# NWC-CUAHSI-Summer-Institute/LGAR-py

Hardware: AMD Instinct MI355X
Metric: column-timesteps/sec (higher is better)
Workload: dtype f32

## Files before the change

lgar_py_amd/csrc/lgar_column.hpp:

```cpp
#pragma once
#include "lgar_geff.hpp"

namespace lgar {

template <typename R> struct Glob {
  R dt_h, initial_psi, pdm, wp_psi, frozen;
  R giuh[LGAR_GMAX];
  int nint, nsub, ng, bottom_mode, closed_form;
  long long iter_cap;
};

#define LGAR_COOP_GROUPS 16
template <typename S, int FMAX, int STRIDE = WAVE> struct FrontsView {
  S *base;
  unsigned char *fl;
  __device__ __forceinline__ S &Z(int i) const { return base[(0 * FMAX + i) * STRIDE]; }
  __device__ __forceinline__ S &TH(int i) const { return base[(1 * FMAX + i) * STRIDE]; }
  __device__ __forceinline__ S &PS(int i) const { return base[(2 * FMAX + i) * STRIDE]; }
  __device__ __forceinline__ S &DZ(int i) const { return base[(3 * FMAX + i) * STRIDE]; }
  __device__ __forceinline__ unsigned char &flag(int i) const { return fl[i * STRIDE]; }
  __device__ __forceinline__ int layer(int i) const { return fl[i * STRIDE] & 0x7f; }
  __device__ __forceinline__ bool bottom(int i) const { return (fl[i * STRIDE] & LGAR_FLAG_BOTTOM) != 0; }
  __device__ __forceinline__ void set_flag(int i, int layer, bool bottom) const {
    fl[i * STRIDE] = (unsigned char)(layer | (bottom ? LGAR_FLAG_BOTTOM : 0));
  }
  __device__ __forceinline__ void copy(int dst, int src) const {
    Z(dst) = Z(src); TH(dst) = TH(src); PS(dst) = PS(src); DZ(dst) = DZ(src);
    fl[dst * STRIDE] = fl[src * STRIDE];
  }
};

constexpr int MODE_LITERAL = 0, MODE_FAST = 1, MODE_MIXED = 3, MODE_COOP = 4, MODE_MIXED_COOP = 6;

template <typename S, int MODE> struct ModeTraits : ScalarKind<S> {
  using K = ScalarKind<S>;
  static constexpr bool literal = MODE == MODE_LITERAL;
  static constexpr bool mixed = MODE == MODE_MIXED || MODE == MODE_MIXED_COOP;
  static constexpr bool coop = MODE == MODE_COOP || MODE == MODE_MIXED_COOP;
  static constexpr bool mixed_f64 = mixed && K::plain_f64;
  static constexpr bool coop_f64 = coop && K::plain_f64;
  static constexpr int pol = (literal && K::f64) ? POL_LIBRARY : (!literal && K::plain_f32) ? POL_RCP32 : mixed_f64 ? POL_MIXED : POL_LEAN;
  static constexpr int stride = coop ? LGAR_COOP_GROUPS : WAVE;
  static constexpr bool giuh_mem = MODE == MODE_MIXED && !K::dual;
  static constexpr bool late_forcing_sums = MODE == MODE_MIXED;
  static constexpr bool fused_walk = !literal && !coop;
};

template <typename S, int NL, int FMAX, int MODE> struct Column {
  using R = real_t<S>;
  using M = ModeTraits<S, MODE>;
  static constexpr int POL = M::pol;
  const ColParams<S, NL> &P;
  const LGAR_KARG Glob<R> *G;
  FrontsView<S, FMAX, M::stride> F;
  int nf;
  int status;
  S ponded_water, previous_precip, ending_volume;
  S giuh_q[LGAR_GMAX];
  static constexpr int DEAD = LGAR_ST_BOTTOM | LGAR_ST_OVERFLOW | LGAR_ST_STRUCT;
  R *giuh_mem = nullptr;
  size_t giuh_stride = 0;
  bool giuh_live = false;
  S k_deepest;
  bool new_front_frozen;
  S memo_theta, memo_g;
  int memo_layer = -1;
  unsigned near_sat_fronts = 0u;
  S post_mass;
  bool post_mass_valid = false;
  bool post_event = false;
  bool psi_rewritten = false;
  S aet_psi_wp_memo;
  bool aet_psi_wp_known = false;
  bool count_geff = false;
  int share_lanes = 0;
  R *xchg = nullptr;
  int coop_rank = 0;
  int cap = FMAX;
  S a_precip, a_pet, a_aet, a_infil, a_runoff, a_perc, a_giuh, a_disch;

  __device__ Column(const ColParams<S, NL> &p, const LGAR_KARG Glob<R> *g, const FrontsView<S, FMAX, M::stride> &f) : P(p), G(g), F(f) {}

  __device__ __forceinline__ S cum_at(int k) const { return sel<S, NL>(P.cum, k); }
  __device__ __forceinline__ S capillary_drive(const LayerK<S> &lk, S theta1, S theta2, int site = 0, CoopRiders *riders = nullptr) {
    (void)site; (void)riders;
    LGAR_MEASURE_POINT(NOGEFF, lk, theta1, theta2)
    LGAR_COUNT_GEFF_CALL(site)
    LGAR_MEASURE_POINT(DUP_GEFF, lk, theta1, theta2)
    if constexpr (M::literal && M::f64) {
      return G->closed_form ? geff_closed<S, POL>(lk, theta1, theta2) : geff_literal<S, POL>(lk, theta1, theta2, G->nint);
    }
    if constexpr (M::dual && M::f64 && !M::literal) {
      if (share_lanes >= 2 && !G->closed_form) return geff_fused<S>(lk, theta1, theta2, G->nint, xchg, share_lanes);
    }
    if constexpr (M::coop_f64 && !M::mixed) {
      if (share_lanes > 1 && !G->closed_form) return geff_fused<S>(lk, theta1, theta2, G->nint, xchg, share_lanes, coop_rank, riders);
    }
    if constexpr (M::coop_f64 && M::mixed) {
      if (share_lanes > 1 && !G->closed_form)
        return geff_mixed_coop(val(lk.alpha), val(lk.n), val(lk.m), val(lk.inv_m), val(lk.inv_n), val(lk.ksat), val(lk.te), val(lk.tr),
                               theta1, theta2, G->nint, xchg, share_lanes, coop_rank);
    }
    if constexpr (M::mixed_f64) {
      if (!G->closed_form)
        return geff_mixed(val(lk.alpha), val(lk.n), val(lk.m), val(lk.inv_m), val(lk.inv_n), val(lk.ksat), val(lk.te), val(lk.tr),
                          theta1, theta2, G->nint);
    }
    return G->closed_form ? geff_closed<S, POL>(lk, theta1, theta2) : geff(lk, theta1, theta2, G->nint);
  }
  __device__ __forceinline__ double capillary_drive_fronts(const LayerK<double> &lk, double theta1, double theta2, double psi1,
                                                           double psi2, double &kr_end) {
    LGAR_MEASURE_POINT(NOGEFF_FRONTS, lk, theta1, theta2, kr_end)
    LGAR_COUNT_GEFF_CALL(1)
    if constexpr (M::coop && M::mixed) {
      if (share_lanes > 1) return geff_mixed_heads<true>(lk, theta1, theta2, psi1, psi2, G->nint, kr_end, xchg, share_lanes, coop_rank);
    }
    return geff_mixed_heads(lk, theta1, theta2, psi1, psi2, G->nint, kr_end);
  }
  __device__ __forceinline__ S cum_prev(int k) const {
    S r = S(R(0.0));
#pragma unroll
    for (int j = 0; j < NL - 1; j++) {
      const S cj = P.cum[j];
      r = choose(k == j + 1, cj, r);
    }
    return r;
  }

  __device__ __forceinline__ bool feq(int a, int b) const {
    return val(F.Z(a)) == val(F.Z(b)) && val(F.PS(a)) == val(F.PS(b)) && val(F.DZ(a)) == val(F.DZ(b));
  }
  __device__ __forceinline__ void fdel(int i) {
    for (int j = i; j < nf - 1; j++) F.copy(j, j + 1);
    nf--;
  }
  __device__ __forceinline__ void range_of(int k, int &lo, int &len) const {
    lo = -1; len = 0;
    for (int i = 0; i < nf; i++)
      if (F.layer(i) == k) { if (len == 0) lo = i; len++; }
  }

  static constexpr int SCAN = 8;
  struct Rows {
    R z[SCAN], th[SCAN];
    int fl[SCAN];
  };
  __device__ __forceinline__ void fetch_rows(Rows &r) const {
#pragma unroll
    for (int q = 0; q < SCAN; q++) {
      r.z[q] = val(F.Z(q));
      r.th[q] = val(F.TH(q));
      r.fl[q] = F.flag(q);
    }
  }

  __device__ __forceinline__ S mass_balance() const {
    S ls[NL];
    if constexpr (M::coop_f64) {
      if (nf <= SCAN) {
        Rows r;
        fetch_rows(r);
#pragma unroll
        for (int j = 0; j < NL; j++) ls[j] = S(R(0.0));
#pragma unroll
        for (int q = 0; q < SCAN; q++) {
          const bool on = q < nf;
          const int lay = r.fl[q] & 0x7f;
          const bool next_same = (q + 1 < nf) && ((r.fl[(q + 1 < SCAN) ? q + 1 : q] & 0x7f) == lay);
          const R dth = next_same ? r.th[q] - r.th[(q + 1 < SCAN) ? q + 1 : q] : r.th[q];
          R base = R(0.0);
#pragma unroll
          for (int j = 1; j < NL; j++) base = choose(lay == j, val(P.cum[j]) - val(P.thick[j]), base);
          const R term = (r.z[q] - base) * dth;
#pragma unroll
          for (int j = 0; j < NL; j++) ls[j] = choose(on && lay == j, ls[j] + term, ls[j]);
        }
        S tot = ls[NL - 1];
#pragma unroll
        for (int j = NL - 2; j >= 0; j--) tot = ls[j] + tot;
        return tot;
      }
    }
    int i = 0;
#pragma unroll
    for (int j = 0; j < NL; j++) {
      S base = (j == 0) ? S(R(0.0)) : P.cum[j] - P.thick[j];
      S sum = S(R(0.0));
      while (i < nf && F.layer(i) == j) {
        bool next_same = (i + 1 < nf) && (F.layer(i + 1) == j);
        S dth = next_same ? (F.TH(i) - F.TH(i + 1)) : F.TH(i);
        sum = sum + (F.Z(i) - base) * dth;
// ... 1051 lines not shown
            riders.n = 1 + k;
            riders.l = le;
            riders.se = se_from_theta(le, th_e);
#pragma unroll
            for (int q = 0; q < LGAR_LMAX; q++) riders.k[q] = R(1.0);
            g = capillary_drive(lk, theta_1, theta_2, 1, &riders);
            ki = riders.k[0];
            if (i == 0 && new_front_frozen) ki = ki * G->frozen;
            fronts_done = true;
          }
        }
        LGAR_MEASURE_POINT(F32_HEADS_FROM_PSI, lk, i, g, ki, fronts_done)
        if (!fronts_done) {
          g = capillary_drive(lk, theta_1, theta_2, 1);
          ki = front_k(i, lk);
        }
        if (is_nan(val(g))) status |= LGAR_ST_NAN;
        S dzdt;
        if (k == 0) {
          dzdt = dv<POL>(S(R(1.0)), delta_theta) * (dv<POL>(lk.ksat * (g + h_p), F.Z(i)) + ki);
        } else {
          S den = S(R(0.0)) + dv<POL>(F.Z(i) - cum_prev(k), ki);
#pragma unroll
          for (int j = 0; j < NL - 1; j++)
            if (j < k) {
              const LayerK<S> lj = pick_static(P, j);
              S kl;
              bool rode = false;
              if constexpr (M::coop_f64 && !M::mixed) {
                if (riders.n > 0) { kl = riders.k[1 + j]; rode = true; }
              }
              if (!rode) {
                S tl = theta_from_h<S, POL>(lj, F.PS(i));
                kl = k_from_se<S, POL>(lj, se_from_theta(lj, tl));
              }
              S pt = (j != 0) ? P.cum[(j > 0) ? j - 1 : 0] : S(R(0.0));
              den = den + dv<POL>(P.cum[j] - pt, kl);
            }
          dzdt = dv<POL>(S(R(1.0)), delta_theta) * (dv<POL>(F.Z(i), den) + dv<POL>(lk.ksat * (g + h_p), F.Z(i)));
        }
        F.DZ(i) = dzdt;
        LGAR_MEASURE_POINT(CLK, 17)
      }
    }
  }

  __device__ __forceinline__ S calc_dry_depth() {
    const LayerK<S> l0 = pick_static(P, 0);
    S delta_theta = l0.te - F.TH(0);
    S tau = G->dt_h * l0.ksat / delta_theta;
    S g = capillary_drive(l0, F.TH(0), l0.te, 2);
    if (is_nan(val(g))) status |= LGAR_ST_NAN;
    S dry = R(0.5) * (tau + sq(tau * tau + R(4.0) * tau * g));
    return mn(P.cum[0], dry);
  }

  __device__ __forceinline__ void create_surficial_front(S dry_depth, S &ponded, S &infiltration) {
    if (nf >= cap) { status |= LGAR_ST_OVERFLOW; return; }
    const LayerK<S> l0 = pick_static(P, 0);
    S cur_theta = F.TH(0);
    S delta_theta = l0.te - cur_theta;
    S theta_new;
    bool to_bottom = false;
    if (val(dry_depth * delta_theta) > val(ponded)) {
      infiltration = ponded;
      theta_new = mn((cur_theta + ponded / dry_depth), l0.te);
      ponded = S(R(0.0));
    } else {
      infiltration = dry_depth * delta_theta;
      ponded = ponded - (dry_depth * delta_theta);
      theta_new = l0.te;
      to_bottom = !(val(dry_depth) < val(P.cum[0]));
    }
    for (int j = nf; j > 0; j--) F.copy(j, j - 1);
    nf++;
    F.Z(0) = dry_depth;
    F.TH(0) = theta_new;
    F.set_flag(0, 0, to_bottom);
    F.PS(0) = h_from_se<S, POL>(l0, se_from_theta(l0, theta_new));
    new_front_frozen = true;
    F.DZ(0) = S(R(0.0));
  }

  __device__ __forceinline__ void insert_water(int fdd, S precip, S &ponded, S &infiltration, S &runoff) {
    const R dt = G->dt_h;
    S h_p = (ponded - precip) * dt;
    if (val(h_p) < R(0.0)) h_p = S(R(0.0));
    const int kfp = F.layer(fdd);
    int lo, len;
    range_of(kfp, lo, len);
    const int nxt_i = lo + 1;
    if (nxt_i >= nf && (nf != NL || G->bottom_mode == 0)) { status |= LGAR_ST_STRUCT; return; }
    const LayerK<S> lk = pick(P, kfp);
    S g = S(R(0.0));
    if (nf != NL) {
      const S theta_1 = F.TH(nxt_i < nf ? nxt_i : nf - 1);
      bool hit = memo_layer == kfp && same_bits(theta_1, memo_theta);
      if constexpr (M::dual) {
        if (share_lanes >= 2) {
          const bool value_hit = memo_layer == kfp && val(theta_1) == val(memo_theta);
          if (any_lane(value_hit && !hit) != 0ull) hit = false;
        }
      }
      if (hit) {
        g = memo_g;
      } else {
        g = capillary_drive(lk, theta_1, lk.te, 3);
        memo_theta = theta_1; memo_g = g; memo_layer = kfp;
      }
    }
    if (is_nan(val(g))) status |= LGAR_ST_NAN | LGAR_ST_NEGBASE;
    S f_p;
    if (kfp == 0) {
      f_p = P.ksat[0] * (R(1.0) + dv<POL>(g + h_p, F.Z(fdd)));
    } else {
      S fd_ksat = lk.ksat * G->frozen;
      S bottom_sum = dv<POL>(F.Z(fdd) - cum_prev(kfp), fd_ksat);
      bottom_sum = bottom_sum + dv<POL>(P.cum[0] - R(0.0), P.ksat[0] * G->frozen);
#pragma unroll
      for (int j = 1; j < NL - 1; j++)
        if (j < kfp) {
          const LayerK<S> lj = pick_static(P, j);
          S tl = theta_from_h<S, POL>(lj, F.PS(fdd));
          S kl = k_from_se<S, POL>(lj, se_from_theta(lj, tl));
          bottom_sum = bottom_sum + dv<POL>(P.cum[j] - P.cum[j - 1], kl);
        }
      f_p = dv<POL>(F.Z(fdd), bottom_sum) + dv<POL>((g + h_p) * fd_ksat, F.Z(fdd));
    }
    S pond_temp = ponded - f_p * dt;
    if (val(pond_temp) < R(0.0)) pond_temp = S(R(0.0));
    S fp_cm = f_p * dt;
    if (G->pdm > R(0.0)) {
      if (val(pond_temp) < G->pdm) {
        infiltration = mn(ponded, fp_cm);
        ponded = ponded - infiltration;
      } else if (val(pond_temp) > G->pdm) {
        ponded = S(G->pdm);
        infiltration = fp_cm;
      }
      S r = pond_temp - G->pdm;
      runoff = (val(r) > R(0.0)) ? r : S(R(0.0));
    } else {
      infiltration = mn(ponded, fp_cm);
      S r = ponded - infiltration;
      ponded = S(G->pdm);
      runoff = (val(r) > R(0.0)) ? r : S(R(0.0));
    }
  }

  __device__ __forceinline__ void init_state() {
    nf = NL;
    status = 0;
    new_front_frozen = false;
#pragma unroll
    for (int k = 0; k < NL; k++) {
      const LayerK<S> lk = pick_static(P, k);
      F.Z(k) = P.cum[k];
      F.TH(k) = theta_from_h<S, POL>(lk, S(G->initial_psi));
      F.PS(k) = S(G->initial_psi);
      if (k == NL - 1) k_deepest = k_from_se<S, POL>(lk, se_from_theta(lk, F.TH(k)));
      F.DZ(k) = S(R(0.0));
      F.set_flag(k, k, true);
    }
    ponded_water = previous_precip = S(R(0.0));
#pragma unroll
    for (int i = 0; i < LGAR_GMAX; i++) giuh_q[i] = S(R(0.0));
    ending_volume = mass_balance();
    drain();
  }

  __device__ __forceinline__ void drain() {
    a_precip = a_pet = a_aet = a_infil = a_runoff = a_perc = a_giuh = a_disch = S(R(0.0));
  }

  __device__ __forceinline__ void forward(S precip, S pet) {
    const R dt = G->dt_h;
    if (is_nan(val(precip)) || is_nan(val(pet))) status |= LGAR_ST_NAN;
    S ending_volume_sub = ending_volume;
    for (int sub = 0; sub < G->nsub; sub++) {
      if (status & DEAD) return;
      new_front_frozen = false;
      post_mass_valid = false;
      S precip_sub = precip * dt;
      S pet_sub = pet * dt;
      S ponded_depth_sub = precip_sub + ponded_water;
      S ponded_water_sub = S(R(0.0)), runoff_sub = S(R(0.0)), infiltration_sub = S(R(0.0)), AET_sub = S(R(0.0));
      const bool create = (val(previous_precip) == R(0.0)) && (val(precip_sub) > R(0.0)) && (val(ponded_water) == R(0.0));
      LGAR_MEASURE_POINT(CLK, 0)
      LGAR_MEASURE_POINT(DUP_FDD)
      const int fdd = free_drainage_front();
      const bool saturated = val(F.TH(0)) >= val(P.te[0]);
      if (val(pet) > R(0.0)) {
        if (!aet_psi_wp_known) {
          aet_psi_wp_memo = aet_psi_wp<S, POL>(pick_static(P, 0), G->wp_psi);
          aet_psi_wp_known = true;
        }
        AET_sub = aet_from_psi_wp<S, POL>(pet, dt, F.PS(0), aet_psi_wp_memo);
      }
      if constexpr (!M::late_forcing_sums) {
        a_precip = a_precip + precip_sub;
        a_pet = a_pet + ((val(pet_sub) > R(0.0)) ? pet_sub : S(R(0.0)));
      }
      const bool inserting = !create && val(ponded_depth_sub) > R(0.0);
      LGAR_MEASURE_POINT(CLK, 1)
      if (inserting) {
        LGAR_ABLATABLE(INSERT, insert_water(fdd, precip_sub, ponded_depth_sub, infiltration_sub, runoff_sub);)
        a_infil = a_infil + infiltration_sub;
        a_runoff = a_runoff + runoff_sub;
        ponded_water_sub = ponded_depth_sub;
      }
      LGAR_MEASURE_POINT(CLK, 2)
      if (!create || !saturated) {
        S perc_sub = S(R(0.0));
        LGAR_ABLATABLE(MOVE, perc_sub = move_wetting_front(create ? S(R(0.0)) : infiltration_sub, AET_sub, ending_volume_sub, fdd);)
        if (!create) a_perc = a_perc + perc_sub;
      }
      if (__builtin_expect(create && !saturated, 0)) {
        S dry_depth = calc_dry_depth();
        create_surficial_front(dry_depth, ponded_depth_sub, infiltration_sub);
        a_infil = a_infil + infiltration_sub;
        post_mass_valid = false;
      }
      if (!inserting) {
        if (val(ponded_depth_sub) < G->pdm) {
          runoff_sub = S(R(0.0));
          ponded_water_sub = ponded_depth_sub;
          ponded_depth_sub = S(R(0.0));
        } else {
          runoff_sub = ponded_depth_sub - G->pdm;
          ponded_depth_sub = S(G->pdm);
          ponded_water_sub = ponded_depth_sub;
          a_runoff = a_runoff + runoff_sub;
        }
      }
      LGAR_MEASURE_POINT(CLK, 5)
      LGAR_ABLATABLE(DZDT, calc_dzdt(ponded_depth_sub);)
      LGAR_MEASURE_POINT(CLK, 6)
      LGAR_MEASURE_POINT(DUP_DZDT, ponded_depth_sub)
      LGAR_MEASURE_POINT(DUP_MB, ending_volume_sub)
      if constexpr (M::fused_walk) {
        if (__builtin_expect(!post_mass_valid, 0)) post_mass = mass_balance();
        ending_volume_sub = post_mass;
      } else {
        ending_volume_sub = mass_balance();
      }
      LGAR_MEASURE_POINT(CLK, 7)
      previous_precip = precip_sub;
      ending_volume = ending_volume_sub;
      if constexpr (M::late_forcing_sums) {
        a_precip = a_precip + precip_sub;
        a_pet = a_pet + ((val(pet_sub) > R(0.0)) ? pet_sub : S(R(0.0)));
      }
      a_aet = a_aet + AET_sub;
      ponded_water = ponded_water_sub;
      if constexpr (M::giuh_mem) {
        if (giuh_live || val(runoff_sub) > R(0.0)) {
          const int ng = G->ng;
          S q[LGAR_GMAX];
#pragma unroll
          for (int i = 0; i < LGAR_GMAX; i++) q[i] = (i < ng) ? S(giuh_mem[(size_t)i * giuh_stride]) : S(R(0.0));
#pragma unroll
          for (int i = 0; i < LGAR_GMAX; i++) if (i < ng) q[i] = q[i] + (G->giuh[i] * runoff_sub);
          const S now = q[0];
          R qsum = R(0.0);
#pragma unroll
          for (int i = 0; i < LGAR_GMAX; i++) {
            const S shifted = (i + 1 < LGAR_GMAX) ? q[(i + 1 < LGAR_GMAX) ? i + 1 : i] : S(R(0.0));
            qsum += val(shifted);
            if (i < ng) giuh_mem[(size_t)i * giuh_stride] = val(shifted);
          }
          giuh_live = qsum > R(0.0);
          a_giuh = a_giuh + now;
          a_disch = a_disch + now;
        }
      } else {
      R qsum = R(0.0);
#pragma unroll
      for (int i = 0; i < LGAR_GMAX; i++) qsum += val(giuh_q[i]);
      if (qsum > R(0.0) || val(runoff_sub) > R(0.0)) {
#pragma unroll
        for (int i = 0; i < LGAR_GMAX; i++) if (i < G->ng) giuh_q[i] = giuh_q[i] + (G->giuh[i] * runoff_sub);
        S now = giuh_q[0];
#pragma unroll
        for (int i = 0; i < LGAR_GMAX - 1; i++) giuh_q[i] = giuh_q[i + 1];
        giuh_q[LGAR_GMAX - 1] = S(R(0.0));
        a_giuh = a_giuh + now;
        a_disch = a_disch + now;
      }
      }
// ... 14 lines not shown
```

lgar_py_amd/csrc/lgar_geff.hpp:

```cpp
#pragma once
#include "lgar_vg.hpp"

namespace lgar {

#define LGAR_COOP_TAB 128
#define LGAR_COOP_TAB_ROW 130
#define LGAR_COOP_PAIR_LANES 12
#ifndef LGAR_DEVSIM
template <int W>
__device__ __forceinline__ void geff_coop_node_rounds(const LayerK<double> &l, double nm1, double half_m, double k_sat1, double k_first,
                                                      double hdh, int nint, int lanes, double *tab, int r) {
  const int stride = W * lanes;
  for (int first = 0; first < nint; first += stride) {
    double h[W], k[W];
    bool ok[W];
#pragma unroll
    for (int u = 0; u < W; u++) {
      const int j = first + r + u * lanes;
      ok[u] = (r < lanes) && (j < nint);
      h[u] = tab[ok[u] ? j : 0];
    }
#pragma unroll
    for (int u = 0; u < W; u++) k[u] = geff_node(l, nm1, half_m, h[u]);
#pragma unroll
// ... 234 lines not shown
}
typedef float f32x2 __attribute__((ext_vector_type(2)));
__device__ __forceinline__ float geff_f32_from_heads(const LayerK<float> &l, float h_i, float h_f, int nint, float *kn_out = nullptr) {
  const float dh = (h_f - h_i) * (1.0f / float(nint));
  const float nm1 = l.n - 1.0f;
  const float hm = -0.5f * l.m;
  const float x0 = l.alpha * h_i, dx = l.alpha * dh, xcut = 0.1f * l.alpha;
  const float tsat = 1.0f - ex2(l.m * -39.863137f);
  const float ksat1 = tsat * tsat;
  auto node = [&](float x) {
    const float lg = lg2(x);
    const float P = ex2(nm1 * lg);
    const float l1 = lg2(__builtin_fmaf(x, P, 1.0f));
    const float sr = ex2(hm * l1);
    const float t = __builtin_fmaf(-P, sr * sr, 1.0f);
    const float k = sr * (t * t);
    return (x < xcut) ? ksat1 : k;
  };
  const int M = nint - 1;
  const int pairs = M >> 1;
#ifndef LGAR_DEVSIM
  const float jf = (x0 - xcut) * __builtin_amdgcn_rcpf(-dx) - 1.5f;
#else
  const float jf = (x0 - xcut) / -dx - 1.5f;
#endif
  int safe = (jf > 0.0f) ? ((jf < float(M)) ? int(jf) : M) : 0;
  safe >>= 1;
  int safe_pairs = pairs;
  if (any_lane(safe < pairs) != 0ull) {
    safe_pairs = 0;
    for (int bit = 64; bit; bit >>= 1) {
      const int cand = safe_pairs + bit;
      if (cand <= pairs && any_lane(safe < cand) == 0ull) safe_pairs = cand;
    }
  }
  const f32x2 dx2 = {dx, dx}, x02 = {x0, x0}, nm12 = {nm1, nm1}, hm2 = {hm, hm};
  const f32x2 one2 = {1.0f, 1.0f}, two2 = {2.0f, 2.0f}, four2 = {4.0f, 4.0f};
  f32x2 ja = {1.0f, 2.0f};
  f32x2 acc = {0.0f, 0.0f}, accb = {0.0f, 0.0f};
#define LGAR_GEFF_PAIR(X, SR, TT)                                              \
  {                                                                            \
    f32x2 lg, P, l1;                                                           \
    lg.x = lg2((X).x); lg.y = lg2((X).y);                                      \
    const f32x2 e0 = nm12 * lg;                                                \
    P.x = ex2(e0.x); P.y = ex2(e0.y);                                          \
    const f32x2 opa = __builtin_elementwise_fma((X), P, one2);                 \
    l1.x = lg2(opa.x); l1.y = lg2(opa.y);                                      \
    const f32x2 e1 = hm2 * l1;                                                 \
    (SR).x = ex2(e1.x); (SR).y = ex2(e1.y);                                    \
    const f32x2 t = __builtin_elementwise_fma(-P, (SR) * (SR), one2);          \
    (TT) = t * t;                                                              \
  }
  int it = 0;
  for (; it + 1 < safe_pairs; it += 2) {
    const f32x2 xa = __builtin_elementwise_fma(ja, dx2, x02);
    const f32x2 xb = __builtin_elementwise_fma(ja + two2, dx2, x02);
    ja = ja + four2;
    f32x2 sa, ta, sb, tb;
    LGAR_GEFF_PAIR(xa, sa, ta)
    acc = __builtin_elementwise_fma(sa, ta, acc);
    LGAR_GEFF_PAIR(xb, sb, tb)
    accb = __builtin_elementwise_fma(sb, tb, accb);
  }
  if (it < safe_pairs) {
    const f32x2 x = __builtin_elementwise_fma(ja, dx2, x02);
    f32x2 sr, tt;
    LGAR_GEFF_PAIR(x, sr, tt)
    acc = __builtin_elementwise_fma(sr, tt, acc);
    it++;
  }
  for (; it < pairs; it++) {
    const float j0 = float(2 * it + 1);
    const f32x2 j2 = {j0, j0 + 1.0f};
    const f32x2 x = __builtin_elementwise_fma(j2, dx2, x02);
    f32x2 sr, tt;
    LGAR_GEFF_PAIR(x, sr, tt)
    sr.x = (x.x < xcut) ? ksat1 : sr.x;
    tt.x = (x.x < xcut) ? 1.0f : tt.x;
    sr.y = (x.y < xcut) ? ksat1 : sr.y;
    tt.y = (x.y < xcut) ? 1.0f : tt.y;
    if (it & 1) accb = __builtin_elementwise_fma(sr, tt, accb);
    else acc = __builtin_elementwise_fma(sr, tt, acc);
  }
#undef LGAR_GEFF_PAIR
  acc = acc + accb;
  float sum = acc.x + acc.y;
  if (M & 1) sum += node(__builtin_fmaf(float(M), dx, x0));
  const float k0 = node(x0), kn = node(l.alpha * h_f);
  if (kn_out != nullptr) *kn_out = kn;
  return fabsf((0.5f * dh) * ((k0 + kn) + 2.0f * sum));
}
template <> __device__ __forceinline__ float geff<float>(const LayerK<float> &l, float theta1, float theta2, int nint) {
  const float se_i = se_from_theta(l, theta1);
  const float se_f = se_from_theta(l, theta2);
  const float inv_alpha = 1.0f / l.alpha;
  auto head = [&](float se) {
    float base = pw(se, -l.inv_m) - 1.0f;
    if (fabsf(base) <= 1e-8f) base = base + 1e-12f;
    return inv_alpha * pw(base, l.inv_n);
  };
  return geff_f32_from_heads(l, head(se_i), head(se_f), nint);
}
template <> __device__ __forceinline__ double geff<double>(const LayerK<double> &l, double t1, double t2, int nint) {
  return geff_fused<double>(l, t1, t2, nint);
}

#define LGAR_LOG2_1EM12 -39.863137138648355
__device__ __forceinline__ void mixed_end(const LayerK<double> &l, double se, double &h, double &kr) {
  const double q = lg2e(se) * l.inv_m;
  const double C = ex2e(q);
  const double omc = 1.0 - C;
  const bool k_nudged = fabs(omc) <= 1e-8;
  const double bk = k_nudged ? omc + 1e-12 : omc;
  const double u = (omc == 0.0) ? LGAR_LOG2_1EM12 : lg2e(bk);
  const double t = 1.0 - ex2e(l.m * u);
  kr = sqrt(se) * (t * t);
  const double bh = omc / C;
  const bool h_nudged = fabs(bh) <= 1e-8;
  double lbh = (omc == 0.0) ? u : u - q;
  if (any_lane((k_nudged || h_nudged) && omc != 0.0) != 0ull) {
    const double own = lg2e(h_nudged ? bh + 1e-12 : bh);
    lbh = ((k_nudged || h_nudged) && omc != 0.0) ? own : lbh;
  }
  h = (1.0 / l.alpha) * ex2e(lbh * l.inv_n);
}
template <bool COOPERATE = false>
__device__ __forceinline__ double geff_mixed_core(const LayerK<double> &l, double h_i, double h_f, double k0, double kn_own, double ksat1,
                                                  int nint, double *tab = nullptr, int lanes = 0, int r = 0) {
  (void)tab; (void)lanes; (void)r;
  const float ksat1f = (float)ksat1;
  const double dh = (h_f - h_i) / double(nint);
  const double x0 = l.alpha * h_i, dx = l.alpha * dh, xcut = 0.1 * l.alpha;
  const double hmd = -0.5 * l.m;
  const float hm = (float)hmd, hm_lo = (float)(hmd - (double)hm);
  const int M = nint - 1;
  const int pairs = M >> 1;
  const double inv_ndx = 1.0 / -dx;
  const double jf = (x0 - xcut) * inv_ndx - 1.5;
  int safe = (jf > 0.0) ? ((jf < double(M)) ? int(jf) : M) : 0;
  safe >>= 1;
  int safe_pairs = pairs;
  if (!COOPERATE && any_lane(safe < pairs) != 0ull) {
    safe_pairs = 0;
    for (int bit = 64; bit; bit >>= 1) {
      const int cand = safe_pairs + bit;
      if (cand <= pairs && any_lane(safe < cand) == 0ull) safe_pairs = cand;
    }
  }
  const float xcutf = (float)xcut;
  const float nf = (float)l.n, nf_lo = (float)(l.n - (double)nf), mmf = (float)(-l.m), mmf_lo = (float)(-l.m - (double)mmf);
  const f32x2 n2 = {nf, nf}, nl2 = {nf_lo, nf_lo}, hm2 = {hm, hm}, hml2 = {hm_lo, hm_lo}, one2 = {1.0f, 1.0f};
  const f32x2 ln2_2 = {0.693147181f, 0.693147181f}, c2_2 = {0.240226507f, 0.240226507f}, c3_2 = {0.0555041087f, 0.0555041087f};
  const f32x2 c4_2 = {0.00961812911f, 0.00961812911f}, c5_2 = {0.00133335581f, 0.00133335581f};
  const f32x2 mm2 = {mmf, mmf}, mml2 = {mmf_lo, mmf_lo}, ilog2 = {1.44269504f, 1.44269504f}, two_ilog2 = {2.88539008f, 2.88539008f};
  const f32x2 half2 = {0.5f, 0.5f};
#define LGAR_GEFFM_PAIR(X, SR, TT, KIND)                                                    \
  {                                                                                         \
     \
    f32x2 lg, r, Lc;                                                                        \
    lg.x = lg2((X).x); lg.y = lg2((X).y);                                                   \
    const f32x2 la = __builtin_elementwise_fma(n2, lg, nl2 * lg);                           \
    r.x = ex2(-la.x); r.y = ex2(-la.y);                                                     \
    const f32x2 c = one2 + r;                                                               \
    const f32x2 rho = r - (c - one2);                                                       \
    Lc.x = lg2(c.x); Lc.y = lg2(c.y);                                                       \
     \
    f32x2 ic = __builtin_elementwise_fma(-ilog2, c, two_ilog2);                             \
    if ((KIND) != 1) { ic.x = fmaxf(ic.x, 0.0f); ic.y = fmaxf(ic.y, 0.0f); }                \
    const f32x2 L = __builtin_elementwise_fma(rho, ic, Lc);                                 \
     \
    const f32x2 E = __builtin_elementwise_fma(mm2, L, mml2 * L);                            \
    const f32x2 e1 = __builtin_elementwise_fma(hm2, la, __builtin_elementwise_fma(hml2, la, half2 * E)); \
    (SR).x = ex2(e1.x); (SR).y = ex2(e1.y);                                                 \
                                                             \
    f32x2 t;                                                                                \
    if ((KIND) == 1) {                                                                      \
      f32x2 p = __builtin_elementwise_fma(c5_2, E, c4_2);                                   \
      p = __builtin_elementwise_fma(p, E, c3_2);                                            \
      p = __builtin_elementwise_fma(p, E, c2_2);                                            \
      p = __builtin_elementwise_fma(p, E, ln2_2);                                           \
      t = -E * p;                                                                           \
    } else if ((KIND) == 2) {                                                               \
      f32x2 w;                                                                              \
      w.x = ex2(E.x); w.y = ex2(E.y);                                                       \
// ... 224 lines not shown
```

lgar_py_amd/csrc/lgar_measure.hpp:

```cpp
#pragma once

__device__ __forceinline__ float opaque(float x) { asm volatile("" : "+v"(x)); return x; }
__device__ __forceinline__ double opaque(double x) { asm volatile("" : "+v"(x)); return x; }

#define LGAR_MEASURE_POINT(NAME, ...) LGAR_POINT_##NAME(__VA_ARGS__)
#define LGAR_ABLATABLE(NAME, ...) LGAR_STMT_##NAME(__VA_ARGS__)

#ifdef LGAR_ABL_NOINSERT
#define LGAR_STMT_INSERT(...)
#else
#define LGAR_STMT_INSERT(...) __VA_ARGS__
#endif
#ifdef LGAR_ABL_NOMOVE
#define LGAR_STMT_MOVE(...)
#else
#define LGAR_STMT_MOVE(...) __VA_ARGS__
#endif
#ifdef LGAR_ABL_NODZDT
#define LGAR_STMT_DZDT(...)
#else
#define LGAR_STMT_DZDT(...) __VA_ARGS__
#endif

#ifdef LGAR_ABL_NOGEFF
#define LGAR_POINT_NOGEFF(lk, theta1, theta2) return theta1 * theta2 + lk.alpha;
#else
#define LGAR_POINT_NOGEFF(lk, theta1, theta2)
#endif
#ifdef LGAR_ABL_NOGEFF
#define LGAR_POINT_NOGEFF_FRONTS(lk, theta1, theta2, kr) { kr = theta1; return theta1 * theta2 + lk.alpha; }
#else
#define LGAR_POINT_NOGEFF_FRONTS(lk, theta1, theta2, kr)
#endif
#ifdef LGAR_COUNT_SITE
#define LGAR_COUNT_IF_SITE(site) if (site == LGAR_COUNT_SITE)
#else
#define LGAR_COUNT_IF_SITE(site)
#endif
#ifdef LGAR_COUNT_MAXLANES
#define LGAR_COUNT_IF_SPARSE if (__builtin_popcountll(any_lane(true)) <= LGAR_COUNT_MAXLANES)
#else
#define LGAR_COUNT_IF_SPARSE
#endif
#ifdef LGAR_COUNT_LANES
#define LGAR_COUNT_WHO count_geff
#else
#define LGAR_COUNT_WHO (count_geff && first_active_lane())
#endif
#define LGAR_COUNT_GEFF_CALL(site) \
  LGAR_COUNT_IF_SITE(site) LGAR_COUNT_IF_SPARSE { if (LGAR_COUNT_WHO) status += (1 << LGAR_ST_STEP_SHIFT); }
#ifdef LGAR_DUP_GEFF
#define LGAR_POINT_DUP_GEFF(lk, theta1, theta2)                                                    \
  if constexpr (!M::dual) {                                                                         \
    const S extra = geff(lk, opaque(theta1), opaque(theta2), G->nint);                             \
    if (val(extra) == R(12345.678)) return extra;  \
  }
#else
#define LGAR_POINT_DUP_GEFF(lk, theta1, theta2)
#endif

#ifdef LGAR_ABL_NOSEARCH
#define LGAR_POINT_NOSEARCH(lk, psi, new_mass) return theta_from_h<S, POL>(lk, psi + new_mass);
#else
#define LGAR_POINT_NOSEARCH(lk, psi, new_mass)
#endif
#ifdef LGAR_DUP_SEARCH
#define LGAR_POINT_DUP_SEARCH(K, lk, psi, new_mass, prior_mass, dth, dthick, dth_k, dthick_k)      \
  if constexpr (!M::dual) {                                                                         \
    const S extra = theta_mass_balance<K>(lk, opaque(psi), opaque(new_mass), opaque(prior_mass), dth, dthick, dth_k, dthick_k); \
    if (val(extra) == R(-1.0)) status |= LGAR_ST_STRUCT;                           \
  }
#else
#define LGAR_POINT_DUP_SEARCH(...)
#endif

#ifdef LGAR_DUP_EVENT
#define LGAR_POINT_DUP_EVENT()                                                                     \
  if (front_event_pending() && val(F.Z(0)) == R(-12345.0)) status |= LGAR_ST_STRUCT;  \
  asm volatile("" ::: "memory");
#else
#define LGAR_POINT_DUP_EVENT()
#endif
#ifdef LGAR_DUP_PSI
#define LGAR_POINT_DUP_PSI() asm volatile("" ::: "memory"); update_psi();
#else
#define LGAR_POINT_DUP_PSI()
#endif
#ifdef LGAR_DUP_FDD
#define LGAR_POINT_DUP_FDD()                                                                       \
  if (free_drainage_front() == 12345) status |= LGAR_ST_STRUCT;                    \
  asm volatile("" ::: "memory");
#else
#define LGAR_POINT_DUP_FDD()
#endif
#ifdef LGAR_DUP_DZDT
#define LGAR_POINT_DUP_DZDT(h_p) asm volatile("" ::: "memory"); calc_dzdt(h_p);
#else
#define LGAR_POINT_DUP_DZDT(h_p)
#endif
#ifdef LGAR_DUP_MB
#define LGAR_POINT_DUP_MB(volume)                                                                  \
  volume = mass_balance();                                                                         \
  asm volatile("" ::: "memory");                                                                   \
  if (val(volume) == R(-1.0)) status |= LGAR_ST_STRUCT;
#else
#define LGAR_POINT_DUP_MB(volume)
#endif

#ifdef LGAR_GEFFM_GENERAL_ONLY
#define LGAR_POINT_GEFFM_GENERAL_ONLY(ser_pairs, dir_pair, pairs) ser_pairs = 0; dir_pair = pairs + 1;
#else
#define LGAR_POINT_GEFFM_GENERAL_ONLY(ser_pairs, dir_pair, pairs)
#endif
static __device__ unsigned long long lgar_dbg_counters[8];
#ifndef LGAR_COUNT_GEFFM_REGIONS
#define LGAR_POINT_GEFFM_REGIONS(a, b, c, d)
#else
#define LGAR_POINT_GEFFM_REGIONS(a, b, c, d)                                                        \
  if (first_active_lane()) {                                                                       \
    atomicAdd(&lgar_dbg_counters[0], (unsigned long long)(a));                                     \
    atomicAdd(&lgar_dbg_counters[1], (unsigned long long)(b));                                     \
    atomicAdd(&lgar_dbg_counters[2], (unsigned long long)(c));                                     \
    atomicAdd(&lgar_dbg_counters[3], (unsigned long long)(d));                                     \
    atomicAdd(&lgar_dbg_counters[4], 1ull);                                                        \
    atomicAdd(&lgar_dbg_counters[5], (unsigned long long)__builtin_popcountll(any_lane(true)));    \
  }
#endif

#ifdef LGAR_CLOCKS
static __device__ unsigned long long lgar_dbg_clk[64];
static __shared__ unsigned long long lgar_dbg_clk_last;
#define LGAR_POINT_CLK(id)                                                                         \
  if (blockIdx.x == 0) {                                                                           \
// ... 60 lines not shown
```

Measured before the change: 12.45 billion.

## Pair idle lanes with geff-needing lanes to split f32 quadrature work

```diff
diff --git a/lgar_py_amd/csrc/lgar_column.hpp b/lgar_py_amd/csrc/lgar_column.hpp
--- a/lgar_py_amd/csrc/lgar_column.hpp
+++ b/lgar_py_amd/csrc/lgar_column.hpp
@@ -81,6 +81,12 @@
 
   __device__ Column(const ColParams<S, NL> &p, const LGAR_KARG Glob<R> *g, const FrontsView<S, FMAX, M::stride> &f) : P(p), G(g), F(f) {}
 
+#ifdef LGAR_NO_PAIRED_GEFF
+  static constexpr bool paired_geff = false;
+#else
+  static constexpr bool paired_geff = M::plain_f32 && !M::literal;
+#endif
+
   __device__ __forceinline__ S cum_at(int k) const { return sel<S, NL>(P.cum, k); }
   __device__ __forceinline__ S capillary_drive(const LayerK<S> &lk, S theta1, S theta2, int site = 0, CoopRiders *riders = nullptr) {
     (void)site; (void)riders;
@@ -107,6 +113,14 @@
                           theta1, theta2, G->nint);
     }
     return G->closed_form ? geff_closed<S, POL>(lk, theta1, theta2) : geff(lk, theta1, theta2, G->nint);
+  }
+  __device__ __forceinline__ S capillary_drive_paired(const LayerK<S> &lk, S theta1, S theta2, bool want, int site) {
+    (void)site;
+    LGAR_MEASURE_POINT(COUNT_IF_PAIRED, want)
+    if (want) { LGAR_COUNT_GEFF_CALL(site) }
+    S h_i = S(R(1.0)), h_f = S(R(1.0));
+    if (want) geff_f32_heads(lk, theta1, theta2, h_i, h_f);
+    return geff_f32_paired(lk, h_i, h_f, G->nint, want);
   }
   __device__ __forceinline__ double capillary_drive_fronts(const LayerK<double> &lk, double theta1, double theta2, double psi1,
                                                            double psi2, double &kr_end) {
@@ -1324,7 +1338,26 @@
     F.DZ(0) = S(R(0.0));
   }
 
-  __device__ __forceinline__ void insert_water(int fdd, S precip, S &ponded, S &infiltration, S &runoff) {
+  __device__ __forceinline__ S insert_water_geff(bool inserting, int fdd) {
+    bool want = false;
+    LayerK<S> lk = pick_static(P, 0);
+    S theta_1 = lk.te;
+    if (inserting) {
+      const int kfp = F.layer(fdd);
+      int lo, len;
+      range_of(kfp, lo, len);
+      const int nxt_i = lo + 1;
+      const bool structural = nxt_i >= nf && (nf != NL || G->bottom_mode == 0);
+      if (!structural && nf != NL) {
+        theta_1 = F.TH(nxt_i < nf ? nxt_i : nf - 1);
+        want = !(memo_layer == kfp && same_bits(theta_1, memo_theta));
+        if (want) lk = pick(P, kfp);
+      }
+    }
+    return capillary_drive_paired(lk, theta_1, lk.te, want, 3);
+  }
+
+  __device__ __forceinline__ void insert_water(int fdd, S precip, S &ponded, S &infiltration, S &runoff, const S *g_ready = nullptr) {
     const R dt = G->dt_h;
     S h_p = (ponded - precip) * dt;
     if (val(h_p) < R(0.0)) h_p = S(R(0.0));
@@ -1347,7 +1380,7 @@
       if (hit) {
         g = memo_g;
       } else {
-        g = capillary_drive(lk, theta_1, lk.te, 3);
+        g = (g_ready != nullptr) ? *g_ready : capillary_drive(lk, theta_1, lk.te, 3);
         memo_theta = theta_1; memo_g = g; memo_layer = kfp;
       }
     }
@@ -1445,8 +1478,16 @@
       }
       const bool inserting = !create && val(ponded_depth_sub) > R(0.0);
       LGAR_MEASURE_POINT(CLK, 1)
+      if constexpr (paired_geff) {
+        if (!G->closed_form) {
+          const S g_insert = insert_water_geff(inserting, fdd);
+          if (inserting) insert_water(fdd, precip_sub, ponded_depth_sub, infiltration_sub, runoff_sub, &g_insert);
+        } else if (inserting) {
+          insert_water(fdd, precip_sub, ponded_depth_sub, infiltration_sub, runoff_sub);
+        }
+      }
       if (inserting) {
-        LGAR_ABLATABLE(INSERT, insert_water(fdd, precip_sub, ponded_depth_sub, infiltration_sub, runoff_sub);)
+        if constexpr (!paired_geff) { LGAR_ABLATABLE(INSERT, insert_water(fdd, precip_sub, ponded_depth_sub, infiltration_sub, runoff_sub);) }
         a_infil = a_infil + infiltration_sub;
         a_runoff = a_runoff + runoff_sub;
         ponded_water_sub = ponded_depth_sub;
diff --git a/lgar_py_amd/csrc/lgar_geff.hpp b/lgar_py_amd/csrc/lgar_geff.hpp
--- a/lgar_py_amd/csrc/lgar_geff.hpp
+++ b/lgar_py_amd/csrc/lgar_geff.hpp
@@ -340,7 +340,6 @@
     if (it & 1) accb = __builtin_elementwise_fma(sr, tt, accb);
     else acc = __builtin_elementwise_fma(sr, tt, acc);
   }
-#undef LGAR_GEFF_PAIR
   acc = acc + accb;
   float sum = acc.x + acc.y;
   if (M & 1) sum += node(__builtin_fmaf(float(M), dx, x0));
@@ -348,7 +347,120 @@
   if (kn_out != nullptr) *kn_out = kn;
   return fabsf((0.5f * dh) * ((k0 + kn) + 2.0f * sum));
 }
-template <> __device__ __forceinline__ float geff<float>(const LayerK<float> &l, float theta1, float theta2, int nint) {
+#ifndef LGAR_DEVSIM
+__device__ __forceinline__ float lane_read(float v, int src) {
+  return __int_as_float(__builtin_amdgcn_ds_bpermute(src << 2, __float_as_int(v)));
+}
+__device__ __forceinline__ int nth_set_lane(unsigned long long m, int r) {
+  int pos = 0;
+#pragma unroll
+  for (int b = 32; b; b >>= 1) {
+    const int c = __builtin_popcountll((m >> pos) & ((1ull << b) - 1ull));
+    if (r >= c) { r -= c; pos += b; }
+  }
+  return pos;
+}
+#endif
+__device__ __forceinline__ float geff_f32_paired(const LayerK<float> &l, float h_i, float h_f, int nint, bool want) {
+#ifndef LGAR_DEVSIM
+  const unsigned long long W = any_lane(want), Fr = any_lane(!want);
+  const int nw = __builtin_popcountll(W);
+  if (nw > __builtin_popcountll(Fr))
+#endif
+  {
+    float g = 0.0f;
+    if (want) g = geff_f32_from_heads(l, h_i, h_f, nint);
+    return g;
+  }
+#ifndef LGAR_DEVSIM
+  if (nw == 0) return 0.0f;
+  const int rank_w = (int)__builtin_amdgcn_mbcnt_hi((unsigned)(W >> 32), __builtin_amdgcn_mbcnt_lo((unsigned)W, 0u));
+  const int rank_f = (int)__builtin_amdgcn_mbcnt_hi((unsigned)(Fr >> 32), __builtin_amdgcn_mbcnt_lo((unsigned)Fr, 0u));
+  const int rank = want ? rank_w : rank_f;
+  const int partner = nth_set_lane(want ? Fr : W, rank);
+  const int lane = (int)__builtin_amdgcn_mbcnt_hi(~0u, __builtin_amdgcn_mbcnt_lo(~0u, 0u));
+  const int src = (!want && rank < nw) ? partner : lane;
+  const float dh = (h_f - h_i) * (1.0f / float(nint));
+  const float tsat = 1.0f - ex2(l.m * -39.863137f);
+  const float x0 = lane_read(l.alpha * h_i, src), dx = lane_read(l.alpha * dh, src);
+  const float nm1 = lane_read(l.n - 1.0f, src), hm = lane_read(-0.5f * l.m, src);
+  const float xcut = lane_read(0.1f * l.alpha, src), ksat1 = lane_read(tsat * tsat, src);
+  const int M = nint - 1;
+  const int pairs = M >> 1;
+  const float jf = (x0 - xcut) * __builtin_amdgcn_rcpf(-dx) - 1.5f;
+  int safe = (jf > 0.0f) ? ((jf < float(M)) ? int(jf) : M) : 0;
+  safe >>= 1;
+  int safe_pairs = pairs;
+  if (any_lane(want && safe < pairs) != 0ull) {
+    safe_pairs = 0;
+    for (int bit = 64; bit; bit >>= 1) {
+      const int cand = safe_pairs + bit;
+      if (cand <= pairs && any_lane(want && safe < cand) == 0ull) safe_pairs = cand;
+    }
+  }
+  const f32x2 dx2 = {dx, dx}, x02 = {x0, x0}, nm12 = {nm1, nm1}, hm2 = {hm, hm};
+  const f32x2 one2 = {1.0f, 1.0f}, four2 = {4.0f, 4.0f}, eight2 = {8.0f, 8.0f};
+  const int q = want ? 0 : 1;
+  const float q2 = want ? 0.0f : 2.0f;
+  f32x2 ja = {1.0f + q2, 2.0f + q2};
+  f32x2 a = {0.0f, 0.0f};
+  const int jsafe = safe_pairs >> 1, jtot = (pairs + 1) >> 1;
+  int j = 0;
+  for (; j + 1 < jsafe; j += 2) {
+    const f32x2 xa = __builtin_elementwise_fma(ja, dx2, x02);
+    const f32x2 xb = __builtin_elementwise_fma(ja + four2, dx2, x02);
+    ja = ja + eight2;
+    f32x2 sa, ta, sb, tb;
+    LGAR_GEFF_PAIR(xa, sa, ta)
+    LGAR_GEFF_PAIR(xb, sb, tb)
+    a = __builtin_elementwise_fma(sa, ta, a);
+    a = __builtin_elementwise_fma(sb, tb, a);
+  }
+  if (j < jsafe) {
+    const f32x2 x = __builtin_elementwise_fma(ja, dx2, x02);
+    f32x2 sr, tt;
+    LGAR_GEFF_PAIR(x, sr, tt)
+    a = __builtin_elementwise_fma(sr, tt, a);
+    j++;
+  }
+  for (; j < jtot; j++) {
+    const int p = q + 2 * j;
+    if (p < pairs) {
+      const float j0 = float(2 * p + 1);
+      const f32x2 j2 = {j0, j0 + 1.0f};
+      const f32x2 x = __builtin_elementwise_fma(j2, dx2, x02);
+      f32x2 sr, tt;
+      LGAR_GEFF_PAIR(x, sr, tt)
+      sr.x = (x.x < xcut) ? ksat1 : sr.x;
+      tt.x = (x.x < xcut) ? 1.0f : tt.x;
+      sr.y = (x.y < xcut) ? ksat1 : sr.y;
+      tt.y = (x.y < xcut) ? 1.0f : tt.y;
+      a = __builtin_elementwise_fma(sr, tt, a);
+    }
+  }
+  const f32x2 accb = {lane_read(a.x, partner), lane_read(a.y, partner)};
+  float g = 0.0f;
+  if (want) {
+    auto node = [&](float x) {
+      const float lg = lg2(x);
+      const float P = ex2(nm1 * lg);
+      const float l1 = lg2(__builtin_fmaf(x, P, 1.0f));
+      const float sr = ex2(hm * l1);
+      const float t = __builtin_fmaf(-P, sr * sr, 1.0f);
+      const float k = sr * (t * t);
+      return (x < xcut) ? ksat1 : k;
+    };
+    const f32x2 acc = a + accb;
+    float sum = acc.x + acc.y;
+    if (M & 1) sum += node(__builtin_fmaf(float(M), dx, x0));
+    const float k0 = node(x0), kn = node(l.alpha * h_f);
+    g = fabsf((0.5f * dh) * ((k0 + kn) + 2.0f * sum));
+  }
+  return g;
+#endif
+}
+#undef LGAR_GEFF_PAIR
+__device__ __forceinline__ void geff_f32_heads(const LayerK<float> &l, float theta1, float theta2, float &h_i, float &h_f) {
   const float se_i = se_from_theta(l, theta1);
   const float se_f = se_from_theta(l, theta2);
   const float inv_alpha = 1.0f / l.alpha;
@@ -357,7 +469,13 @@
     if (fabsf(base) <= 1e-8f) base = base + 1e-12f;
     return inv_alpha * pw(base, l.inv_n);
   };
-  return geff_f32_from_heads(l, head(se_i), head(se_f), nint);
+  h_i = head(se_i);
+  h_f = head(se_f);
+}
+template <> __device__ __forceinline__ float geff<float>(const LayerK<float> &l, float theta1, float theta2, int nint) {
+  float h_i, h_f;
+  geff_f32_heads(l, theta1, theta2, h_i, h_f);
+  return geff_f32_from_heads(l, h_i, h_f, nint);
 }
 template <> __device__ __forceinline__ double geff<double>(const LayerK<double> &l, double t1, double t2, int nint) {
   return geff_fused<double>(l, t1, t2, nint);
diff --git a/lgar_py_amd/csrc/lgar_measure.hpp b/lgar_py_amd/csrc/lgar_measure.hpp
--- a/lgar_py_amd/csrc/lgar_measure.hpp
+++ b/lgar_py_amd/csrc/lgar_measure.hpp
@@ -49,6 +49,14 @@
 #endif
 #define LGAR_COUNT_GEFF_CALL(site) \
   LGAR_COUNT_IF_SITE(site) LGAR_COUNT_IF_SPARSE { if (LGAR_COUNT_WHO) status += (1 << LGAR_ST_STEP_SHIFT); }
+#ifdef LGAR_COUNT_PAIRED
+#define LGAR_POINT_COUNT_IF_PAIRED(want) if (__builtin_popcountll(any_lane(want)) <= __builtin_popcountll(any_lane(!(want))))
+#else
+#define LGAR_POINT_COUNT_IF_PAIRED(want)
+#endif
+#if defined(LGAR_ABL_NOGEFF) || defined(LGAR_DUP_GEFF) || defined(LGAR_ABL_NOINSERT) || defined(LGAR_F32_HEADS_FROM_PSI)
+#define LGAR_NO_PAIRED_GEFF
+#endif
 #ifdef LGAR_DUP_GEFF
 #define LGAR_POINT_DUP_GEFF(lk, theta1, theta2)                                                    \
   if constexpr (!M::dual) {                                                                         \
```

New measurement: 12.50 billion, median of 6. Within noise of the previous version (+0.4%).
